# MattPlumlee/outerbase

Hardware: AMD Instinct MI355X
Metric: fit+predict points/sec, d=20 n=1e+06 p=4096 (higher is better)
Workload: dtype f64; 1 GPU; BASELINE.json configs[2]: d=20 n=1000000 (1000000 rows on each of 1 GPU(s)) p=4096, mat25, 40 knots/dim, fit (Gram+Cholesky) + predict on n fresh rows; backend=newton, rows_total=1000000, rows_per_gpu=1000000, d=20, p=4096, terms_nnz=12177, basis_columns=101, parallelism=one rank: nothing to exchange (y standardised first, one B^T y pass)

## Files before the change

outerbase_amd/csrc/kernels_gram_panel.hip:

```cpp
#include <algorithm>
#include <map>
#include <mutex>
#include <tuple>

#include <memory>
#include "obhip_internal.h"
#include "device_common.h"

namespace obhip {

namespace {

constexpr int kGT = 128;
constexpr int kCR = 16;
constexpr int kTP = 2 * 128 + 16;
constexpr int kTB = 65;

template <int W2>
__global__ void __launch_bounds__(256)
k_materialize_rows(const double *__restrict__ bm, const double *__restrict__ scale,
                   const uint32_t *__restrict__ ucol, int Mu, uint64_t Mc,
                   const uint32_t *__restrict__ colsw, int W2rt, uint64_t p_pad,
                   double *__restrict__ out) {
  extern __shared__ double lds[];
  double *tb = lds + (size_t)Mu * kTileRows;
  const int lane = threadIdx.x & 63;
  const int wave = __builtin_amdgcn_readfirstlane(threadIdx.x >> 6);
  const uint64_t tile = blockIdx.x;
  stage_tile<false, false>(lds, bm + tile * Mc * kTileRows, ucol, Mu, threadIdx.x, 256);
  __syncthreads();
  const double s = scale[tile * kTileRows + lane];
  double *mytb = tb + wave * 32 * kTB;
  const int ngroups = (int)(p_pad / 64);
  for (int g = wave; g < ngroups; g += 4) {
    const int k0 = g * 64;
    uint32_t cw[W2 > 0 ? W2 : 1];
    if constexpr (W2 > 0) load_cw(cw, colsw, k0 + lane);
#pragma unroll
    for (int h = 0; h < 2; ++h) {
#pragma unroll
      for (int t = 0; t < 32; ++t) {
        double v;
        if constexpr (W2 > 0)
          v = term_prod_rl<W2>(lds, cw, h * 32 + t, lane, s);
        else
          v = term_prod_mem(lds, colsw + (size_t)(k0 + h * 32 + t) * W2rt, W2rt, lane, s);
        mytb[t * kTB + lane] = v;
      }
      asm volatile("s_waitcnt lgkmcnt(0)" ::: "memory");
      double *dst = out + (tile * kTileRows + (lane >> 5)) * p_pad + k0 + h * 32 + (lane & 31);
      const double *src = mytb + (lane & 31) * kTB + (lane >> 5);
#pragma unroll 8
      for (int i = 0; i < 32; ++i) dst[(size_t)(2 * i) * p_pad] = src[2 * i];
      asm volatile("s_waitcnt lgkmcnt(0)" ::: "memory");
    }
  }
}

__device__ __forceinline__ void lds_dma_1k(const char *gbase , uint32_t voff,
                                           uint32_t lds_addr ) {
#pragma clang diagnostic push
#pragma clang diagnostic ignored "-Winline-asm"
  asm volatile("s_mov_b32 m0, %2\n\ts_nop 0\n\tglobal_load_lds_dwordx4 %0, %1"
               :: "v"(voff), "s"(gbase), "s"(lds_addr) : "memory", "m0");
#pragma clang diagnostic pop
}

template <int OFF>
__device__ __forceinline__ double lds_rd(uint32_t addr) {
  double v;
  asm volatile("ds_read_b64 %0, %1 offset:%2" : "=v"(v) : "v"(addr), "n"(OFF));
  return v;
}

__device__ __forceinline__ void lds_wait12(double (&a)[4], double (&b)[4][4]) {
  asm volatile("s_waitcnt lgkmcnt(8)"
               : "+v"(a[0]), "+v"(a[1]), "+v"(a[2]), "+v"(a[3]), "+v"(b[0][0]), "+v"(b[0][1]),
                 "+v"(b[0][2]), "+v"(b[0][3]), "+v"(b[1][0]), "+v"(b[1][1]), "+v"(b[1][2]),
                 "+v"(b[1][3]));
}
template <int KEEP>
__device__ __forceinline__ void lds_wait8(double (&b)[4][4]) {
  asm volatile("s_waitcnt lgkmcnt(%8)"
               : "+v"(b[2][0]), "+v"(b[2][1]), "+v"(b[2][2]), "+v"(b[2][3]), "+v"(b[3][0]),
                 "+v"(b[3][1]), "+v"(b[3][2]), "+v"(b[3][3])
               : "n"(KEEP));
}
template <int OFF>
__device__ __forceinline__ void lds_rd_h0(uint32_t aaddr, const uint32_t (&baddr)[4],
                                          double (&a)[4], double (&b)[4][4]) {
  a[0] = lds_rd<OFF>(aaddr);
  a[1] = lds_rd<OFF + 128>(aaddr);
  a[2] = lds_rd<OFF + 256>(aaddr);
  a[3] = lds_rd<OFF + 384>(aaddr);
#pragma unroll
  for (int r = 0; r < 4; ++r) {
    b[0][r] = lds_rd<OFF>(baddr[r]);
    b[1][r] = lds_rd<OFF + 128>(baddr[r]);
  }
}
template <int OFF>
__device__ __forceinline__ void lds_rd_h1(const uint32_t (&baddr)[4], double (&b)[4][4]) {
#pragma unroll
  for (int r = 0; r < 4; ++r) {
    b[2][r] = lds_rd<OFF + 256>(baddr[r]);
    b[3][r] = lds_rd<OFF + 384>(baddr[r]);
  }
}

constexpr int kAtbGram = 0, kAtbNorm = 1, kAtbStore = 2;
__host__ __device__ inline uint64_t atb_task(uint64_t I, uint64_t J, uint64_t y, uint64_t type = 0) {
  return I | (J << 24) | (y << 48) | (type << 62);
}
constexpr uint64_t kAtbNoTask = ~0ull;
__device__ __forceinline__ uint32_t atb_wave_code(uint32_t type, int wave) {
  constexpr uint32_t W = 0x80u;
  const uint32_t t0 = (W | 0x08u) | (W | 0x2cu) << 8 | (W | 0x19u) << 16 | (W | 0x3du) << 24;
  const uint32_t t1 = 0x00u | 0x24u << 8 | 0x35u << 16 | 0x4au << 24;
  const uint32_t t2 = 0x24u | 0x35u << 8 | 0x4au << 16 | 0x6eu << 24;
  const uint32_t t3 = 0x35u | 0x4au << 8 | 0x6eu << 16 | 0x7fu << 24;
  const uint32_t tab = type == 0 ? t0 : (type == 1 ? t1 : (type == 2 ? t2 : t3));
  return (tab >> (8 * wave)) & 0xffu;
}

template <int MODE, bool DBG>
__global__ void __launch_bounds__(256, 2)
k_atb_dma2(const double *__restrict__ A, uint64_t ldA, const double *__restrict__ Bm, uint64_t ldB,
           int nb, int npairs, uint64_t ntiles, uint64_t split_base ,
           int tri ,
           const uint64_t *__restrict__ tasks, double *__restrict__ part, uint64_t ldo,
           unsigned long long *dbgout) {
  extern __shared__ double T[];
  constexpr int tszb = kCR * kTP * 8;
  unsigned long long st0 = 0, sr0 = 0;
  if constexpr (DBG) {
    st0 = __builtin_amdgcn_s_memtime();
    sr0 = __builtin_amdgcn_s_memrealtime();
  }
  const int tid = threadIdx.x;
  const int lane = tid & 63;
  const int wave = __builtin_amdgcn_readfirstlane(tid >> 6);

  const uint64_t task = tasks[blockIdx.x];
  if (task == kAtbNoTask) return;
  const int I = (int)(task & 0xffffff), J = (int)((task >> 24) & 0xffffff), ysplit = (int)((task >> 48) & 0x3fff);
  const uint32_t wcode = atb_wave_code(MODE == kAtbGram ? (uint32_t)(task >> 62) : 0u, wave);

  uint64_t t0, t1;
  if constexpr (MODE == kAtbGram) {
    const uint64_t y = (uint64_t)ysplit, rem = (uint64_t)tri;
    t0 = y * split_base + min(y, rem);
    t1 = t0 + split_base + (y < rem ? 1 : 0);
  } else {
    t0 = 0;
    t1 = tri ? min(ntiles, (uint64_t)(J + 1) * (kGT / kTileRows)) : ntiles;
  }
  const int nchunks = (int)(t1 > t0 ? (t1 - t0) * (kTileRows / kCR) : 0);

  const uint32_t ldsT = (uint32_t)(uintptr_t)(__attribute__((address_space(3))) double *)T;
  const uint32_t lds0 = ldsT + wave * kTP * 8;
  const uint32_t voff = lane * 16;
  const char *gA = (const char *)(A + (t0 * kTileRows + wave) * ldA + (uint64_t)I * kGT);
  const char *gB = (const char *)(Bm + (t0 * kTileRows + wave) * ldB + (uint64_t)J * kGT);
  const uint64_t pitch4 = 4 * ldA * sizeof(double), pitch16 = 4 * pitch4;
  const uint64_t pitch4b = MODE == kAtbGram ? pitch4 : 4 * ldB * sizeof(double), pitch16b = 4 * pitch4b;
  const int rot = nchunks > 0 ? ((I + J) & 7) % nchunks : 0;
  auto issue = [&](int ch, int buf) {
    const uint32_t l = lds0 + buf * tszb;
    int cr = ch + rot;
    cr = cr >= nchunks ? cr - nchunks : cr;
    const char *a = gA + (uint64_t)cr * pitch16, *b = gB + (uint64_t)cr * pitch16b;
#pragma unroll
    for (int q = 0; q < 4; ++q) {
      lds_dma_1k(a + q * pitch4, voff, l + q * 4 * kTP * 8);
      lds_dma_1k(b + q * pitch4b, voff, l + q * 4 * kTP * 8 + kGT * 8);
    }
  };

  const int wm = (int)((wcode >> 4) & 1), wn = (int)((wcode >> 5) & 1);
  const int acol = (int)(wcode & 3) * 64, bcol = (int)((wcode >> 2) & 3) * 64;
  const int mk = lane >> 4, mblk = (lane >> 2) & 3, me = lane & 3;
  double acc[4][4][4];
#pragma unroll
  for (int i = 0; i < 4; ++i)
#pragma unroll
    for (int j = 0; j < 4; ++j)
#pragma unroll
      for (int r = 0; r < 4; ++r) acc[i][j][r] = 0.0;
  const uint32_t aaddr = ldsT + (mk * kTP + acol + mblk * 4 + me) * 8;
  uint32_t baddr[4];
#pragma unroll
  for (int r = 0; r < 4; ++r)
    baddr[r] = ldsT + (mk * kTP + bcol + ((mblk + r) & 3) * 4 + me) * 8;
  auto mfma_half = [&](const double (&a)[4], const double (&b)[4][4], int j0) {
#pragma unroll
    for (int i = 0; i < 4; ++i)
#pragma unroll
      for (int j = j0; j < j0 + 2; ++j)
#pragma unroll
        for (int r = 0; r < 4; ++r)
          acc[i][j][r] = __builtin_amdgcn_mfma_f64_4x4x4f64(a[i], b[j][r], acc[i][j][r], 0, 0, 0);
  };

  if (nchunks > 0) issue(0, 0);
  asm volatile("s_waitcnt vmcnt(0)" ::: "memory");
  __builtin_amdgcn_s_barrier();
  unsigned long long sr1 = 0, sr2 = 0;
  if constexpr (DBG) sr1 = __builtin_amdgcn_s_memrealtime();
  double a0[4], b0[4][4], a1[4], b1[4][4];
  constexpr int stp = 4 * kTP * 8;

#define OB_STEP(cur_a, cur_b, nxt_a, nxt_b, NEXT_OFF, HAS_NEXT)                              \
  lds_wait12(cur_a, cur_b);                                                               \
  if (HAS_NEXT) lds_rd_h0<NEXT_OFF>(aaddr, baddr, nxt_a, nxt_b);                             \
  mfma_half(cur_a, cur_b, 0);                                                                \
  lds_wait8<(HAS_NEXT) ? 12 : 0>(cur_b);                                                     \
  if (HAS_NEXT) lds_rd_h1<NEXT_OFF>(baddr, nxt_b);                                           \
  mfma_half(cur_a, cur_b, 2);

#define OB_CHUNK_BODY2(BUF)                                                                  \
  {                                                                                          \
    constexpr int ob = (BUF) * tszb;                                                         \
    if (c + 1 < nchunks) issue(c + 1, (BUF) ^ 1);                \
    lds_rd_h0<ob>(aaddr, baddr, a0, b0);                                                     \
    lds_rd_h1<ob>(baddr, b0);                                                                \
    OB_STEP(a0, b0, a1, b1, ob + stp, true)                                                  \
    OB_STEP(a1, b1, a0, b0, ob + 2 * stp, true)                                              \
    OB_STEP(a0, b0, a1, b1, ob + 3 * stp, true)                                              \
    OB_STEP(a1, b1, a0, b0, 0, false)                                                        \
    asm volatile("s_waitcnt vmcnt(0)" ::: "memory");     \
    __builtin_amdgcn_s_barrier();                                                            \
    ++c;                                                                                     \
  }

  for (int c = 0; c < nchunks;) {
    OB_CHUNK_BODY2(0)
    if (c >= nchunks) break;
    OB_CHUNK_BODY2(1)
  }
#undef OB_CHUNK_BODY2
#undef OB_STEP
  if constexpr (DBG) sr2 = __builtin_amdgcn_s_memrealtime();

  if constexpr (MODE == kAtbGram) {
    const int sel = (int)(wcode >> 6);
    const int oi = sel == 1 ? J : I, oj = sel == 0 ? I : J;
    const int slot = oi * nb - oi * (oi - 1) / 2 + (oj - oi);
    double *out = part + ((uint64_t)ysplit * npairs + slot) * (kGT * kGT);
#pragma unroll
    for (int i = 0; i < 4; ++i)
#pragma unroll
      for (int j = 0; j < 4; ++j)
#pragma unroll
        for (int r = 0; r < 4; ++r) {
          const int row = wm * 64 + i * 16 + mblk * 4 + mk;
          const int col = wn * 64 + j * 16 + ((mblk + r) & 3) * 4 + me;
          out[row * kGT + col] = acc[i][j][r];
        }
  } else if constexpr (MODE == kAtbStore) {
    double *out = part + ((uint64_t)I * kGT) * ldo + (uint64_t)J * kGT;
#pragma unroll
    for (int i = 0; i < 4; ++i)
#pragma unroll
      for (int j = 0; j < 4; ++j)
#pragma unroll
        for (int r = 0; r < 4; ++r) {
          const int row = wm * 64 + i * 16 + mblk * 4 + mk;
          const int col = wn * 64 + j * 16 + ((mblk + r) & 3) * 4 + me;
          out[(uint64_t)row * ldo + col] = acc[i][j][r];
        }
  } else {
    double *red = T;
#pragma unroll
    for (int i = 0; i < 4; ++i) {
      double s = 0.0;
#pragma unroll
      for (int j = 0; j < 4; ++j)
#pragma unroll
        for (int r = 0; r < 4; ++r) s = fma(acc[i][j][r], acc[i][j][r], s);
      s += __shfl_xor(s, 1, 64);
      s += __shfl_xor(s, 2, 64);
      if (me == 0) red[wn * kGT + wm * 64 + i * 16 + mblk * 4 + mk] = s;
    }
    __syncthreads();
    if (tid < kGT) part[(uint64_t)J * ldo + (uint64_t)I * kGT + tid] = red[tid] + red[kGT + tid];
  }
  if constexpr (DBG) {
    const unsigned which = blockIdx.x == 7 ? 1u : blockIdx.x == gridDim.x / 2 + 7 ? 0u
                           : blockIdx.x + 512 - 7 == gridDim.x - (gridDim.x % 512 ? gridDim.x % 512 : 0) ? 2u : 3u;
    if (dbgout && which < 3 && tid == 0) {
      dbgout[3 * which] = __builtin_amdgcn_s_memtime() - st0;
      dbgout[3 * which + 1] = __builtin_amdgcn_s_memrealtime() - sr0;
      dbgout[3 * which + 2] = nchunks;
    }
    const bool mid0 = blockIdx.x == gridDim.x / 2 + 7, mid1 = blockIdx.x == gridDim.x / 2 + 7 + 512;
    if (dbgout && (mid0 || mid1) && tid == 0) {
      asm volatile("s_waitcnt vmcnt(0)" ::: "memory");
      unsigned long long *o = dbgout + 9 + (mid1 ? 4 : 0);
      o[0] = sr0;
      o[1] = sr1;
      o[2] = sr2;
      o[3] = __builtin_amdgcn_s_memrealtime();
    }
  }
}

constexpr int kXcd = 8, kSq = 8;
struct GramUnit {
  int bi, bj, y, size;
};
void gram_units(int nb, int nsplit, bool diag4, std::vector<GramUnit> &units) {
  const int nsq = (nb + kSq - 1) / kSq;
  for (int y = 0; y < nsplit; ++y)
    for (int bi = 0; bi < nsq; ++bi)
      for (int bj = bi; bj < nsq; ++bj) {
        int size = 0;
        for (int i = bi * kSq; i < std::min(nb, (bi + 1) * kSq); ++i)
          for (int j = std::max(i, bj * kSq); j < std::min(nb, (bj + 1) * kSq); ++j)
            if (!(i == j && diag4 && i / 4 * 4 + 3 < nb && i % 4 == 3)) ++size;
        if (size) units.push_back({bi, bj, y, size});
      }
}
uint64_t gram_xcd_blocks(int nb, int nsplit, bool diag4, bool continuous) {
  std::vector<GramUnit> units;
  gram_units(nb, 1, diag4, units);
  uint64_t per_split = 0;
  for (const GramUnit &u : units) per_split += (uint64_t)u.size;
  if (continuous) return (per_split * (uint64_t)nsplit + kXcd - 1) / kXcd;
  std::vector<int> sizes;
  for (int y = 0; y < nsplit; ++y)
    for (const GramUnit &u : units) sizes.push_back(u.size);
  std::stable_sort(sizes.begin(), sizes.end(), [](int a, int b) { return a > b; });
  uint64_t load[kXcd] = {0};
  for (int s : sizes) {
    int k = 0;
    for (int q = 1; q < kXcd; ++q)
      if (load[q] < load[k]) k = q;
    load[k] += (uint64_t)s;
  }
  return *std::max_element(load, load + kXcd);
}
void build_task_order(int nb, int nsplit, bool diag4, bool continuous, std::vector<uint64_t> &tab) {
  typedef GramUnit Unit;
  std::vector<Unit> units;
  gram_units(nb, nsplit, diag4, units);
  if (!continuous)
    std::stable_sort(units.begin(), units.end(), [](const Unit &a, const Unit &b) { return a.size > b.size; });
  uint64_t total = 0;
  for (const Unit &u : units) total += (uint64_t)u.size;
  const uint64_t run = (total + kXcd - 1) / kXcd;
  uint64_t dealt = 0;
  std::vector<std::vector<uint64_t>> seq(kXcd);
  for (const Unit &u : units) {
    int k = 0;
    for (int q = 1; q < kXcd; ++q)
      if (seq[q].size() < seq[k].size()) k = q;
    if (continuous) {
      for (int i = u.bi * kSq; i < std::min(nb, (u.bi + 1) * kSq); ++i)
        for (int j = std::max(i, u.bj * kSq); j < std::min(nb, (u.bj + 1) * kSq); ++j) {
          if (i == j && diag4) {
            const int g0 = i / 4 * 4;
            if (g0 + 3 < nb) {
              if (i - g0 < 3) seq[(dealt++) / run].push_back(atb_task(i, i + 1, u.y, 1 + (i - g0)));
              continue;
            }
          }
          seq[(dealt++) / run].push_back(atb_task(i, j, u.y));
        }
      continue;
    }
    for (int i = u.bi * kSq; i < std::min(nb, (u.bi + 1) * kSq); ++i)
      for (int j = std::max(i, u.bj * kSq); j < std::min(nb, (u.bj + 1) * kSq); ++j) {
        if (i == j && diag4) {
          const int g0 = i / 4 * 4;
          if (g0 + 3 < nb) {
            if (i - g0 < 3) seq[k].push_back(atb_task(i, i + 1, u.y, 1 + (i - g0)));
            continue;
          }
        }
        seq[k].push_back(atb_task(i, j, u.y));
      }
  }
  size_t len = 0;
  for (auto &q : seq) len = std::max(len, q.size());
  tab.assign(len * kXcd, kAtbNoTask);
  for (int k = 0; k < kXcd; ++k)
    for (size_t m = 0; m < seq[k].size(); ++m) tab[m * kXcd + k] = seq[k][m];
}

template <int W2>
int run_materialize(const obhip_basis &b, obhip_terms &t, double *d_B) {
  const size_t lds = (t.Mu * kTileRows + 4 * 32 * kTB) * sizeof(double);
  OB_TRY(ensure_dyn_lds((const void *)k_materialize_rows<W2>, lds));
  hipLaunchKernelGGL(k_materialize_rows<W2>, dim3((unsigned)(b.n_pad / kTileRows)), dim3(256), lds,
                     cur_stream(), b.bm.p, b.scale.p, t.ucol.p, (int)t.Mu, b.md.Mc,
                     (const uint32_t *)t.cols.p, (int)(t.W / 2), t.p_pad, d_B);
  OB_HIP(hipGetLastError());
  return 0;
}

}

bool gram_panel_supports(const obhip_basis &b, const obhip_terms &t) {
  const size_t need = (size_t)b.n_pad * t.p_pad * sizeof(double);
  if (b.bmat.n * sizeof(double) >= need) return true;
  if (getenv("OBHIP_GRAM_CHUNK_ROWS")) return false;
  size_t free_b = 0, total_b = 0;
  if (hipMemGetInfo(&free_b, &total_b) != hipSuccess) return false;
  return need <= free_b / 2;
}

namespace {

struct RowView {
  obhip_basis v;
  RowView(const obhip_basis &b, uint64_t tile0, uint64_t ntiles) {
    v.model = b.model;
    v.d = b.d;
    v.device = b.device;
    v.md.Mc = b.md.Mc;
    v.n_pad = ntiles * kTileRows;
    const uint64_t r0 = tile0 * kTileRows;
    v.n = r0 >= b.n ? 0 : std::min<uint64_t>(v.n_pad, b.n - r0);
    v.bm.p = b.bm.p + tile0 * b.md.Mc * kTileRows;
    v.scale.p = b.scale.p + r0;
  }
  ~RowView() {
    v.bm.p = nullptr;
    v.scale.p = nullptr;
  }
};

int materialize_any(const obhip_basis &b, obhip_terms &t, double *d_B, GramFuse *fuse = nullptr) {
  if (t.Mu > 280 || getenv("OBHIP_FORCE_GENERIC")) return launch_materialize_generic(b, t, d_B);
  static const bool lane_row = getenv("OBHIP_MATERIALIZE_LANE_ROW") != nullptr;
  if (!lane_row && materialize_tl_supports(t)) {
    const bool f = fuse && fuse->y && fuse->g && !fuse->done;
    OB_TRY(launch_materialize_tl(b, t, d_B, f ? fuse->y : nullptr, f ? fuse->g : nullptr));
    if (f) fuse->done = true;
    return 0;
  }
  switch (t.W / 2) {
    case 1: return run_materialize<1>(b, t, d_B);
    case 2: return run_materialize<2>(b, t, d_B);
    case 3: return run_materialize<3>(b, t, d_B);
    case 4: return run_materialize<4>(b, t, d_B);
    default: return run_materialize<0>(b, t, d_B);
  }
}

int gram_of_staged(obhip_basis &b, const double *d_B, uint64_t ntiles, obhip_terms &t,
                   const GramSink &sink, bool accumulate, bool last) {
  const bool dbg = getenv("OBHIP_GRAM_DBG") && atoi(getenv("OBHIP_GRAM_DBG")) != 0;
  const int nb = (int)((t.p + kGT - 1) / kGT);
  const int npairs = nb * (nb + 1) / 2;
  const int ncu = device_cus(b.device);
  const bool diag4 = !(getenv("OBHIP_GRAM_DIAG4") && atoi(getenv("OBHIP_GRAM_DIAG4")) == 0);
  const uint64_t bps = (uint64_t)npairs - (diag4 ? (uint64_t)(nb / 4) : 0);
  const uint64_t slots = 2 * (uint64_t)ncu;
  uint64_t nsplit = 1;
  const uint64_t max_split = std::max<uint64_t>(
      1, std::min<uint64_t>({64, ntiles / 8, (4ull << 30) / ((uint64_t)npairs * kGT * kGT * 8)}));
  double bestc = 1e300;
  bool continuous = false;
  const uint64_t xslots = slots / kXcd;
  static std::mutex split_mu;
  static std::map<std::tuple<int, uint64_t, uint64_t, uint64_t, bool>, std::pair<uint64_t, bool>> split_cache;
  const auto split_key = std::make_tuple(nb, ntiles, max_split, slots, diag4);
  bool cached = false;
  {
    std::lock_guard<std::mutex> lk(split_mu);
    auto it = split_cache.find(split_key);
    if (it != split_cache.end()) {
      nsplit = it->second.first;
      continuous = it->second.second;
      cached = true;
    }
  }
  for (uint64_t ns = 1; !cached && ns <= max_split; ++ns) {
    const uint64_t blocks = ns * bps;
    for (int mode = 0; mode < 2; ++mode) {
      const uint64_t per = gram_xcd_blocks(nb, (int)ns, diag4, mode == 1);
      const uint64_t full = per / xslots, tail = per % xslots;
      const double rounds = (double)full + (tail == 0 ? 0.0 : (2 * tail <= xslots ? 0.6 : 1.0));
      double cost = rounds * ((double)ntiles / (double)ns + 1.0) + 0.0022 * (double)blocks;
      if (mode == 1) cost *= 1.03;
      if (cost < bestc - 1e-9) {
        bestc = cost;
        nsplit = ns;
        continuous = mode == 1;
      }
    }
  }
  if (!cached) {
    std::lock_guard<std::mutex> lk(split_mu);
    split_cache[split_key] = std::make_pair(nsplit, continuous);
  }
  if (const char *e = getenv("OBHIP_GRAM_NSPLIT")) nsplit = std::max<uint64_t>(1, std::min<uint64_t>(max_split, atoi(e)));
  if (const char *e = getenv("OBHIP_GRAM_CONTINUOUS")) continuous = atoi(e) != 0;
  double *part = nullptr;
  OB_TRY(b.workspace((size_t)nsplit * npairs * kGT * kGT * sizeof(double) + 256, (void **)&part));
  unsigned long long *dbgout =
      dbg ? (unsigned long long *)(part + (size_t)nsplit * npairs * kGT * kGT) : nullptr;
  if (b.gram_pairs_nb != nb || b.gram_pairs_ns != (int)nsplit || b.gram_pairs_diag4 != diag4 ||
      b.gram_pairs_cont != continuous) {
    std::vector<uint64_t> tab;
    build_task_order(nb, (int)nsplit, diag4, continuous, tab);
    b.gram_pairs_diag4 = diag4;
    b.gram_pairs_cont = continuous;
    OB_TRY(b.gram_pairs.upload(tab.data(), tab.size()));
    b.gram_pairs_nb = nb;
    b.gram_pairs_ns = (int)nsplit;
  }
  const unsigned nblocks = (unsigned)b.gram_pairs.n;
  const size_t lds = (size_t)2 * kCR * kTP * sizeof(double);
  {
    ProfScope ps("gram");
    if (dbg) {
      OB_TRY(ensure_dyn_lds((const void *)k_atb_dma2<kAtbGram, true>, lds));
      hipLaunchKernelGGL((k_atb_dma2<kAtbGram, true>), dim3(nblocks), dim3(256), lds, cur_stream(), d_B,
                         t.p_pad, d_B, t.p_pad, nb, npairs, ntiles, ntiles / nsplit, (int)(ntiles % nsplit), b.gram_pairs.p, part,
                         (uint64_t)0, dbgout);
    } else {
      OB_TRY(ensure_dyn_lds((const void *)k_atb_dma2<kAtbGram, false>, lds));
      hipLaunchKernelGGL((k_atb_dma2<kAtbGram, false>), dim3(nblocks), dim3(256), lds, cur_stream(),
                         d_B, t.p_pad, d_B, t.p_pad, nb, npairs, ntiles, ntiles / nsplit, (int)(ntiles % nsplit), b.gram_pairs.p, part,
                         (uint64_t)0, nullptr);
    }
    OB_HIP(hipGetLastError());
  }
  if (dbgout) {
    unsigned long long h[17];
    OB_HIP(hipMemcpy(h, dbgout, sizeof(h), hipMemcpyDeviceToHost));
    fprintf(stderr, "[gram dbg] middle-round block: first chunk %.2f us, loop %.2f us, stores %.2f us; the block one round "
                    "on starts %.2f us after this one ended (its first chunk %.2f us)\n",
            0.01 * (double)(h[10] - h[9]), 0.01 * (double)(h[11] - h[10]), 0.01 * (double)(h[12] - h[11]),
            0.01 * (double)((long long)h[13] - (long long)h[12]), 0.01 * (double)(h[14] - h[13]));
    fprintf(stderr, "[gram dbg] clock of a block of the first / middle / last round: %.0f / %.0f / %.0f MHz\n",
            h[4] ? 100.0 * h[3] / h[4] : 0.0, h[1] ? 100.0 * h[0] / h[1] : 0.0, h[7] ? 100.0 * h[6] / h[7] : 0.0);
    fprintf(stderr,
            "[gram dbg] one block: %llu shader-clock ticks in %llu x 10 ns -> %.0f MHz, %.0f ticks "
            "per 16-row chunk (8192 = matrix pipe saturated by two blocks)\n",
            h[0], h[1], h[1] ? 100.0 * h[0] / h[1] : 0.0, h[2] ? (double)h[0] / h[2] : 0.0);
  }
  return launch_gram_reduce(part, npairs, (int)nsplit, nb, (int)t.p, sink, accumulate, last);
}

}

int launch_materialize_rows(const obhip_basis &b, obhip_terms &t, double *d_B, GramFuse *fuse) {
  OB_TRY(t.prepare(b.md.cap, b.md.dims_h));
  ProfScope ps("materialize_B");
  return materialize_any(b, t, d_B, fuse);
}

int ensure_bmat(obhip_basis &b, obhip_terms &t, GramFuse *fuse) {
  if (b.bmat_terms == t.uid && t.uid != 0) return 0;
  OB_TRY(t.prepare(b.md.cap, b.md.dims_h));
  if (!gram_panel_supports(b, t))
    return fail(OBHIP_ERR_INVALID, "not enough free HBM for the n x p design matrix");
  const size_t need = (size_t)b.n_pad * t.p_pad;
  if (b.bmat.n < need) OB_TRY(b.bmat.alloc(need));
  b.bmat_terms = 0;
  OB_TRY(launch_materialize_rows(b, t, b.bmat.p, fuse));
  b.bmat_terms = t.uid;
  return 0;
}

int launch_gram_panel(const obhip_basis &bc, obhip_terms &t, const GramSink &sink, GramFuse *fuse) {
  obhip_basis &b = const_cast<obhip_basis &>(bc);
  const uint64_t ntiles = b.n_pad / kTileRows;
  if (gram_panel_supports(b, t)) {
    OB_TRY(ensure_bmat(b, t, fuse));
    return gram_of_staged(b, b.bmat.p, ntiles, t, sink, false, true);
  }
  size_t free_b = 0, total_b = 0;
  OB_HIP(hipMemGetInfo(&free_b, &total_b));
  const size_t row_bytes = (size_t)t.p_pad * kTileRows * sizeof(double);
  uint64_t ctiles = std::min<size_t>(free_b / 4, (size_t)16 << 30) / row_bytes;
  if (const char *e = getenv("OBHIP_GRAM_CHUNK_ROWS")) ctiles = (uint64_t)atoll(e) / kTileRows;
  ctiles = std::max<uint64_t>(ctiles, 1);
  ctiles = std::min(ctiles, ntiles);
  if ((size_t)ctiles * row_bytes > free_b)
    return fail(OBHIP_ERR_HIP, "not enough free HBM for even one row chunk of the design matrix");
  b.bmat_terms = 0;
  if (b.bmat.n < (size_t)ctiles * kTileRows * t.p_pad) OB_TRY(b.bmat.alloc((size_t)ctiles * kTileRows * t.p_pad));
  static const bool overlap = getenv("OBHIP_GRAM_OVERLAP") && atoi(getenv("OBHIP_GRAM_OVERLAP")) != 0;
  if (overlap && ctiles < ntiles) {
    DevBuf<double> second;
    OB_TRY(second.alloc((size_t)ctiles * kTileRows * t.p_pad));
    hipStream_t mainst = cur_stream(), side = nullptr;
    OB_HIP(hipStreamCreateWithFlags(&side, hipStreamNonBlocking));
    hipEvent_t ev0, evM[2], evG[2];
    OB_HIP(hipEventCreateWithFlags(&ev0, hipEventDisableTiming));
    for (int i = 0; i < 2; ++i) {
      OB_HIP(hipEventCreateWithFlags(&evM[i], hipEventDisableTiming));
      OB_HIP(hipEventCreateWithFlags(&evG[i], hipEventDisableTiming));
    }
    OB_HIP(hipEventRecord(ev0, mainst));
    OB_HIP(hipStreamWaitEvent(side, ev0, 0));
    int rc = 0;
    uint64_t c = 0;
    for (uint64_t t0 = 0; t0 < ntiles && rc == 0; t0 += ctiles, ++c) {
      const uint64_t nt = std::min(ctiles, ntiles - t0);
      const int buf = (int)(c & 1);
      double *Bp = buf ? second.p : b.bmat.p;
      RowView view(b, t0, nt);
      if (c >= 2) (void)hipStreamWaitEvent(side, evG[buf], 0);
      set_cur_stream(side);
      {
        ProfScope ps("materialize_B");
        rc = materialize_any(view.v, t, Bp);
      }
      (void)hipEventRecord(evM[buf], side);
      set_cur_stream(mainst);
      if (rc) break;
      (void)hipStreamWaitEvent(mainst, evM[buf], 0);
      rc = gram_of_staged(b, Bp, nt, t, sink, t0 != 0, t0 + nt >= ntiles);
      (void)hipEventRecord(evG[buf], mainst);
    }
    (void)hipStreamSynchronize(side);
    (void)hipStreamSynchronize(mainst);
    (void)hipEventDestroy(ev0);
    for (int i = 0; i < 2; ++i) {
      (void)hipEventDestroy(evM[i]);
      (void)hipEventDestroy(evG[i]);
    }
    (void)hipStreamDestroy(side);
    return rc;
  }
  for (uint64_t t0 = 0; t0 < ntiles; t0 += ctiles) {
    const uint64_t nt = std::min(ctiles, ntiles - t0);
    RowView view(b, t0, nt);
    {
      ProfScope ps("materialize_B");
      OB_TRY(materialize_any(view.v, t, b.bmat.p));
    }
    OB_TRY(gram_of_staged(b, b.bmat.p, nt, t, sink, t0 != 0, t0 + nt >= ntiles));
  }
  return 0;
}

int launch_atb(int mode, const double *A, uint64_t ldA, uint64_t M, const double *Bm, uint64_t ldB,
               uint64_t N, uint64_t K, bool tri, double *out, uint64_t ldo) {
  if (M % kGT || N % kGT || K % kTileRows)
    return fail(OBHIP_ERR_INVALID, "launch_atb: sizes must be padded to the tile");
  const uint64_t mt = M / kGT, nt = N / kGT;
  if (mt >= (1ull << 24) || nt >= (1ull << 24)) return fail(OBHIP_ERR_INVALID, "launch_atb: too many tiles");
  constexpr size_t kAtbCache = 8;
  using Tab = std::shared_ptr<DevBuf<uint64_t>>;
  static std::mutex mu;
  static std::map<std::tuple<int, uint64_t, uint64_t>, Tab> cache;
  static std::vector<std::tuple<int, uint64_t, uint64_t>> lru;
  int dev = 0;
  (void)hipGetDevice(&dev);
  Tab dtabp, victim;
  int victim_dev = dev;
  {
    std::lock_guard<std::mutex> lk(mu);
    const auto key = std::make_tuple(dev, mt, nt);
    lru.erase(std::remove(lru.begin(), lru.end(), key), lru.end());
    lru.push_back(key);
    if (lru.size() > kAtbCache) {
      auto it = cache.find(lru.front());
      if (it != cache.end()) {
        victim = std::move(it->second);
        victim_dev = std::get<0>(lru.front());
        cache.erase(it);
      }
      lru.erase(lru.begin());
    }
    Tab &slot = cache[key];
    if (!slot) {
      std::vector<std::vector<uint64_t>> seq(kXcd);
      for (uint64_t bj = 0; bj * kSq < nt; ++bj)
        for (uint64_t bi = 0; bi * kSq < mt; ++bi) {
          int k = 0;
          for (int q = 1; q < kXcd; ++q)
            if (seq[q].size() < seq[k].size()) k = q;
          for (uint64_t i = bi * kSq; i < std::min(mt, (bi + 1) * kSq); ++i)
            for (uint64_t j = bj * kSq; j < std::min(nt, (bj + 1) * kSq); ++j) seq[k].push_back(atb_task(i, j, 0));
        }
      size_t len = 0;
      for (auto &q : seq) len = std::max(len, q.size());
      std::vector<uint64_t> tab(len * kXcd, kAtbNoTask);
      for (int k = 0; k < kXcd; ++k)
        for (size_t m = 0; m < seq[k].size(); ++m) tab[m * kXcd + k] = seq[k][m];
      slot = std::make_shared<DevBuf<uint64_t>>();
      const int rc = slot->upload(tab.data(), tab.size());
      if (rc) {
        cache.erase(key);
        lru.pop_back();
        return rc;
      }
    }
    dtabp = slot;
  }
  if (victim) {
    if (victim_dev != dev) (void)hipSetDevice(victim_dev);
    (void)hipDeviceSynchronize();
    victim.reset();
    if (victim_dev != dev) (void)hipSetDevice(dev);
  }
  DevBuf<uint64_t> &dtab = *dtabp;
  const size_t ntasks = dtab.n;
  const size_t lds = (size_t)2 * kCR * kTP * sizeof(double);
  const uint64_t ktiles = K / kTileRows;
  if (mode == kAtbNorm) {
    OB_TRY(ensure_dyn_lds((const void *)k_atb_dma2<kAtbNorm, false>, lds));
    hipLaunchKernelGGL((k_atb_dma2<kAtbNorm, false>), dim3((unsigned)ntasks), dim3(256), lds,
                       cur_stream(), A, ldA, Bm, ldB, 0, 0, ktiles, ktiles, tri ? 1 : 0, dtab.p, out,
                       ldo, nullptr);
  } else if (mode == kAtbStore) {
    OB_TRY(ensure_dyn_lds((const void *)k_atb_dma2<kAtbStore, false>, lds));
    hipLaunchKernelGGL((k_atb_dma2<kAtbStore, false>), dim3((unsigned)ntasks), dim3(256), lds,
                       cur_stream(), A, ldA, Bm, ldB, 0, 0, ktiles, ktiles, tri ? 1 : 0, dtab.p, out,
                       ldo, nullptr);
  } else {
    return fail(OBHIP_ERR_INVALID, "launch_atb: unknown mode");
  }
  OB_HIP(hipGetLastError());
  return 0;
}

}
```

Baseline: 4.159 million points/s.

## Skip redundant lower-triangle MFMAs in packed diagonal Gram tiles

For Gram tasks that pack four diagonal tile pairs into one block, each wave now gets a role that computes only the upper-triangle MFMAs it owns, plus a few extra rows to rebalance work across waves. It mirrors the needed diagonal entries on store. The split-count cost model is also told how much work this saves. This cuts matrix-pipe work on diagonal blocks, at the price of a second specialised inner loop, more code and register pressure, and a complex ownership mapping guarded by compile-time coverage checks.

```diff
diff --git a/outerbase_amd/csrc/kernels_gram_panel.hip b/outerbase_amd/csrc/kernels_gram_panel.hip
--- a/outerbase_amd/csrc/kernels_gram_panel.hip
+++ b/outerbase_amd/csrc/kernels_gram_panel.hip
@@ -113,7 +113,7 @@
   return I | (J << 24) | (y << 48) | (type << 62);
 }
 constexpr uint64_t kAtbNoTask = ~0ull;
-__device__ __forceinline__ uint32_t atb_wave_code(uint32_t type, int wave) {
+__host__ __device__ constexpr uint32_t atb_wave_code(uint32_t type, int wave) {
   constexpr uint32_t W = 0x80u;
   const uint32_t t0 = (W | 0x08u) | (W | 0x2cu) << 8 | (W | 0x19u) << 16 | (W | 0x3du) << 24;
   const uint32_t t1 = 0x00u | 0x24u << 8 | 0x35u << 16 | 0x4au << 24;
@@ -123,12 +123,179 @@
   return (tab >> (8 * wave)) & 0xffu;
 }
 
+constexpr int kTriMain = 0, kTriD2 = 1, kTriD4 = 2, kTriO10 = 3, kTriO12 = 4;
+constexpr int kTriLen13 = 44, kTriLen2 = 52;
+__host__ __device__ constexpr bool tri_is_d(int kind) { return kind == kTriD2 || kind == kTriD4; }
+__host__ __device__ constexpr bool tri_d_own(int i, int j, int r) { return i < j || (i == j && r < 3); }
+__host__ __device__ constexpr int tri_extra_rows(int kind) { return kind == kTriD2 ? 2 : (kind == kTriD4 ? 4 : 0); }
+__host__ __device__ constexpr bool tri_o_keeps(int kind, int i, int j) {
+  return j >= 2 || (j == 1 && (kind == kTriO12 || i >= 2));
+}
+__host__ __device__ constexpr uint32_t tri_role_byte(int kind, int src = 0, int i0 = 0, int j = 0) {
+  return (uint32_t)kind | (uint32_t)src << 3 | (uint32_t)(i0 >> 1) << 4 | (uint32_t)j << 5;
+}
+__host__ __device__ constexpr uint32_t tri_role(uint32_t type, int wave) {
+  const uint32_t t1 = tri_role_byte(kTriD2, 0, 0, 0) | tri_role_byte(kTriO10) << 8 |
+                      tri_role_byte(kTriD2, 0, 2, 0) << 16 | tri_role_byte(kTriD2, 0, 0, 1) << 24;
+  const uint32_t t2 = tri_role_byte(kTriO12) | tri_role_byte(kTriD4, 0, 0, 0) << 8 |
+                      tri_role_byte(kTriD4, 1, 0, 0) << 16 | tri_role_byte(kTriO12) << 24;
+  const uint32_t t3 = tri_role_byte(kTriD2, 1, 0, 0) | tri_role_byte(kTriD2, 1, 2, 0) << 8 |
+                      tri_role_byte(kTriO10) << 16 | tri_role_byte(kTriD2, 1, 0, 1) << 24;
+  const uint32_t tab = type == 0 ? 0u : (type == 1 ? t1 : (type == 2 ? t2 : t3));
+  return (tab >> (8 * wave)) & 0xffu;
+}
+__host__ __device__ constexpr int tri_role_mfmas(int kind) {
+  int n = 0;
+  for (int i = 0; i < 4; ++i)
+    for (int j = 0; j < 4; ++j)
+      for (int r = 0; r < 4; ++r) n += tri_is_d(kind) ? (tri_d_own(i, j, r) ? 1 : 0) : (tri_o_keeps(kind, i, j) ? 1 : 0);
+  return n + 4 * tri_extra_rows(kind);
+}
+static_assert(tri_role_mfmas(kTriD2) == kTriLen13 && tri_role_mfmas(kTriO10) == 40, "types 1, 3: 44 44 44 40");
+static_assert(tri_role_mfmas(kTriD4) == kTriLen2 && tri_role_mfmas(kTriO12) == 48, "type 2: 48 52 52 48");
+__host__ __device__ constexpr bool tri_cover_ok(uint32_t type, int want_mfmas) {
+  int cnt[2][32][32] = {}, want[2][32][32] = {};
+  int mfmas = 0;
+  for (int w = 0; w < 4; ++w) {
+    const uint32_t code = atb_wave_code(type, w), role = tri_role(type, w);
+    const int sel = (int)(code >> 6), wm = (int)((code >> 4) & 1), wn = (int)((code >> 5) & 1);
+    const int kind = (int)(role & 7);
+    if (sel > 1 || kind == kTriMain) return false;
+    if (tri_is_d(kind) != ((code & 3) == ((code >> 2) & 3))) return false;
+    mfmas += tri_role_mfmas(kind);
+    for (int br = 0; br < 16; ++br)
+      for (int bc = 0; bc < 16; ++bc)
+        if (wn * 16 + bc >= wm * 16 + br) ++want[sel][wm * 16 + br][wn * 16 + bc];
+    for (int i = 0; i < 4; ++i)
+      for (int j = 0; j < 4; ++j)
+        for (int r = 0; r < 4; ++r)
+          for (int blk = 0; blk < 4; ++blk) {
+            if (!(tri_is_d(kind) ? tri_d_own(i, j, r) : tri_o_keeps(kind, i, j))) continue;
+            const int gr = wm * 16 + i * 4 + blk, gc = wn * 16 + j * 4 + ((blk + r) & 3);
+            if (gc >= gr)
+              ++cnt[sel][gr][gc];
+            else if (i == j && r == 1 && blk == 3)
+              ++cnt[sel][gc][gr];
+          }
+    if (tri_is_d(kind)) {
+      const int src = (int)((role >> 3) & 1), i0 = (int)((role >> 4) & 1) * 2, ej = (int)((role >> 5) & 1);
+      for (int k = 0; k < tri_extra_rows(kind); ++k)
+        for (int r = 0; r < 4; ++r)
+          for (int blk = 0; blk < 4; ++blk) ++cnt[src][(i0 + k) * 4 + blk][16 + ej * 4 + ((blk + r) & 3)];
+    }
+  }
+  for (int s = 0; s < 2; ++s)
+    for (int a = 0; a < 32; ++a)
+      for (int b = 0; b < 32; ++b)
+        if (cnt[s][a][b] != want[s][a][b]) return false;
+  return mfmas == want_mfmas;
+}
+static_assert(tri_role(0, 0) == kTriMain && tri_role(0, 1) == kTriMain && tri_role(0, 2) == kTriMain &&
+                  tri_role(0, 3) == kTriMain,
+              "a whole tile pair (type 0) has no roles");
+static_assert(tri_cover_ok(1, 3 * 36 + 64) && tri_cover_ok(2, 2 * 36 + 2 * 64) && tri_cover_ok(3, 3 * 36 + 64),
+              "role tables of the packed diagonal blocks");
+
+struct TriOps {
+  double a[4], b[4][4], ea[4], eb[4];
+};
+template <int KIND>
+struct TriCut {
+  static constexpr bool D = tri_is_d(KIND);
+  static constexpr int nea = tri_extra_rows(KIND);
+  static constexpr int n0 = D ? 11 : 12, n1 = D ? 8 + nea : 4;
+  static_assert(n0 <= 15 && n1 <= 15, "lgkmcnt holds 4 bits");
+};
+template <int KIND, int OFF>
+__device__ __forceinline__ void tri_rd_h0(uint32_t aaddr, const uint32_t (&baddr)[4], TriOps &o) {
+  if constexpr (TriCut<KIND>::D) {
+#pragma unroll
+    for (int r = 0; r < 3; ++r) o.b[0][r] = lds_rd<OFF>(baddr[r]);
+#pragma unroll
+    for (int r = 0; r < 4; ++r) o.b[1][r] = lds_rd<OFF + 128>(baddr[r]);
+#pragma unroll
+    for (int r = 0; r < 4; ++r) o.b[2][r] = lds_rd<OFF + 256>(baddr[r]);
+  } else {
+    o.a[0] = lds_rd<OFF>(aaddr);
+    o.a[1] = lds_rd<OFF + 128>(aaddr);
+    o.a[2] = lds_rd<OFF + 256>(aaddr);
+    o.a[3] = lds_rd<OFF + 384>(aaddr);
+#pragma unroll
+    for (int r = 0; r < 4; ++r) o.b[1][r] = lds_rd<OFF + 128>(baddr[r]);
+#pragma unroll
+    for (int r = 0; r < 4; ++r) o.b[2][r] = lds_rd<OFF + 256>(baddr[r]);
+  }
+}
+template <int KIND, int OFF>
+__device__ __forceinline__ void tri_rd_h1(const uint32_t (&baddr)[4], uint32_t eaaddr,
+                                          const uint32_t (&ebaddr)[4], TriOps &o) {
+#pragma unroll
+  for (int r = 0; r < 4; ++r) o.b[3][r] = lds_rd<OFF + 384>(baddr[r]);
+  if constexpr (TriCut<KIND>::D) {
+    o.ea[0] = lds_rd<OFF>(eaaddr);
+    o.ea[1] = lds_rd<OFF + 128>(eaaddr);
+    if constexpr (TriCut<KIND>::nea == 4) {
+      o.ea[2] = lds_rd<OFF + 256>(eaaddr);
+      o.ea[3] = lds_rd<OFF + 384>(eaaddr);
+    }
+#pragma unroll
+    for (int r = 0; r < 4; ++r) o.eb[r] = lds_rd<OFF>(ebaddr[r]);
+  }
+}
+__device__ __forceinline__ void tri_tie(double &x) { asm volatile("" : "+v"(x)); }
+template <int KIND, int HALF, int KEEP>
+__device__ __forceinline__ void tri_wait(TriOps &o) {
+  asm volatile("s_waitcnt lgkmcnt(%0)" ::"n"(KEEP));
+  constexpr bool D = TriCut<KIND>::D;
+  if constexpr (HALF == 0) {
+    if constexpr (!D) {
+#pragma unroll
+      for (int i = 0; i < 4; ++i) tri_tie(o.a[i]);
+    }
+#pragma unroll
+    for (int j = D ? 0 : 1; j < 3; ++j)
+#pragma unroll
+      for (int r = 0; r < 4; ++r)
+        if (!(D && j == 0 && r == 3)) tri_tie(o.b[j][r]);
+  } else {
+#pragma unroll
+    for (int r = 0; r < 4; ++r) tri_tie(o.b[3][r]);
+    if constexpr (D) {
+#pragma unroll
+      for (int k = 0; k < TriCut<KIND>::nea; ++k) tri_tie(o.ea[k]);
+#pragma unroll
+      for (int r = 0; r < 4; ++r) tri_tie(o.eb[r]);
+    }
+  }
+}
+template <int KIND, int HALF>
+__device__ __forceinline__ void tri_mfma(const TriOps &o, double (&acc)[4][4][4], double (&xacc)[4][4]) {
+  constexpr bool D = TriCut<KIND>::D;
+#pragma unroll
+  for (int j = HALF == 0 ? 0 : 3; j < (HALF == 0 ? 3 : 4); ++j)
+#pragma unroll
+    for (int i = 0; i < 4; ++i)
+#pragma unroll
+      for (int r = 0; r < 4; ++r) {
+        if (D ? tri_d_own(i, j, r) : tri_o_keeps(KIND, i, j))
+          acc[i][j][r] = __builtin_amdgcn_mfma_f64_4x4x4f64(D ? o.b[i][0] : o.a[i], o.b[j][r], acc[i][j][r], 0, 0, 0);
+      }
+  if constexpr (D && HALF == 1) {
+#pragma unroll
+    for (int k = 0; k < TriCut<KIND>::nea; ++k)
+#pragma unroll
+      for (int r = 0; r < 4; ++r)
+        xacc[k][r] = __builtin_amdgcn_mfma_f64_4x4x4f64(o.ea[k], o.eb[r], xacc[k][r], 0, 0, 0);
+  }
+}
+
 template <int MODE, bool DBG>
 __global__ void __launch_bounds__(256, 2)
 k_atb_dma2(const double *__restrict__ A, uint64_t ldA, const double *__restrict__ Bm, uint64_t ldB,
            int nb, int npairs, uint64_t ntiles, uint64_t split_base ,
            int tri ,
            const uint64_t *__restrict__ tasks, double *__restrict__ part, uint64_t ldo,
+           int diagtri ,
            unsigned long long *dbgout) {
   extern __shared__ double T[];
   constexpr int tszb = kCR * kTP * 8;
@@ -145,6 +312,7 @@
   if (task == kAtbNoTask) return;
   const int I = (int)(task & 0xffffff), J = (int)((task >> 24) & 0xffffff), ysplit = (int)((task >> 48) & 0x3fff);
   const uint32_t wcode = atb_wave_code(MODE == kAtbGram ? (uint32_t)(task >> 62) : 0u, wave);
+  const uint32_t role = MODE == kAtbGram && diagtri ? tri_role((uint32_t)(task >> 62), wave) : 0u;
 
   uint64_t t0, t1;
   if constexpr (MODE == kAtbGram) {
@@ -210,6 +378,95 @@
   double a0[4], b0[4][4], a1[4], b1[4][4];
   constexpr int stp = 4 * kTP * 8;
 
+  bool tri_done = false;
+  if constexpr (MODE == kAtbGram) {
+    auto tri_run = [&](auto kind_c) {
+      constexpr int KIND = decltype(kind_c)::value;
+      constexpr bool D = TriCut<KIND>::D;
+      constexpr int nea = TriCut<KIND>::nea, n0 = TriCut<KIND>::n0, n1 = TriCut<KIND>::n1;
+      const int src = (int)((role >> 3) & 1), ei0 = (int)((role >> 4) & 1) * 2, ej = (int)((role >> 5) & 1);
+      const uint32_t eaaddr = ldsT + (mk * kTP + src * kGT + ei0 * 16 + mblk * 4 + me) * 8;
+      uint32_t ebaddr[4];
+#pragma unroll
+      for (int r = 0; r < 4; ++r)
+        ebaddr[r] = ldsT + (mk * kTP + src * kGT + 64 + ej * 16 + ((mblk + r) & 3) * 4 + me) * 8;
+      double tacc[4][4][4], xacc[4][4];
+#pragma unroll
+      for (int i = 0; i < 4; ++i)
+#pragma unroll
+        for (int j = 0; j < 4; ++j) {
+          xacc[i][j] = 0.0;
+#pragma unroll
+          for (int r = 0; r < 4; ++r) tacc[i][j][r] = 0.0;
+        }
+      TriOps o0, o1;
+#define OB_TRI_STEP(cur, nxt, NEXT_OFF, HAS_NEXT)                                            \
+  tri_wait<KIND, 0, n1>(cur);                                                                \
+  if (HAS_NEXT) tri_rd_h0<KIND, NEXT_OFF>(aaddr, baddr, nxt);                                \
+  tri_mfma<KIND, 0>(cur, tacc, xacc);                                                        \
+  tri_wait<KIND, 1, (HAS_NEXT) ? n0 : 0>(cur);                                               \
+  if (HAS_NEXT) tri_rd_h1<KIND, NEXT_OFF>(baddr, eaaddr, ebaddr, nxt);                       \
+  tri_mfma<KIND, 1>(cur, tacc, xacc);
+#define OB_TRI_CHUNK(BUF)                                                                    \
+  {                                                                                          \
+    constexpr int ob = (BUF) * tszb;                                                         \
+    if (c + 1 < nchunks) issue(c + 1, (BUF) ^ 1);                                            \
+    tri_rd_h0<KIND, ob>(aaddr, baddr, o0);                                                   \
+    tri_rd_h1<KIND, ob>(baddr, eaaddr, ebaddr, o0);                                          \
+    OB_TRI_STEP(o0, o1, ob + stp, true)                                                      \
+    OB_TRI_STEP(o1, o0, ob + 2 * stp, true)                                                  \
+    OB_TRI_STEP(o0, o1, ob + 3 * stp, true)                                                  \
+    OB_TRI_STEP(o1, o0, 0, false)                                                            \
+    asm volatile("s_waitcnt vmcnt(0)" ::: "memory");                                         \
+    __builtin_amdgcn_s_barrier();                                                            \
+    ++c;                                                                                     \
+  }
+      for (int c = 0; c < nchunks;) {
+        OB_TRI_CHUNK(0)
+        if (c >= nchunks) break;
+        OB_TRI_CHUNK(1)
+      }
+#undef OB_TRI_CHUNK
+#undef OB_TRI_STEP
+      const int sel = (int)(wcode >> 6);
+      const int ot = sel == 1 ? J : I;
+      double *out = part + ((uint64_t)ysplit * npairs + (ot * nb - ot * (ot - 1) / 2)) * (kGT * kGT);
+#pragma unroll
+      for (int i = 0; i < 4; ++i)
+#pragma unroll
+        for (int j = 0; j < 4; ++j)
+#pragma unroll
+          for (int r = 0; r < 4; ++r) {
+            if (!(D ? tri_d_own(i, j, r) : tri_o_keeps(KIND, i, j))) continue;
+            const int row = wm * 64 + i * 16 + mblk * 4 + mk;
+            const int col = wn * 64 + j * 16 + ((mblk + r) & 3) * 4 + me;
+            out[row * kGT + col] = tacc[i][j][r];
+            if (D && i == j && r == 1 && mblk == 3) out[col * kGT + row] = tacc[i][j][r];
+          }
+      if constexpr (D) {
+        const int xt = src ? J : I;
+        double *xout = part + ((uint64_t)ysplit * npairs + (xt * nb - xt * (xt - 1) / 2)) * (kGT * kGT);
+#pragma unroll
+        for (int k = 0; k < nea; ++k)
+#pragma unroll
+          for (int r = 0; r < 4; ++r) {
+            const int row = (ei0 + k) * 16 + mblk * 4 + mk;
+            const int col = 64 + ej * 16 + ((mblk + r) & 3) * 4 + me;
+            xout[row * kGT + col] = xacc[k][r];
+          }
+      }
+    };
+    if (role != 0) {
+      switch (role & 7) {
+        case kTriD2: tri_run(std::integral_constant<int, kTriD2>()); break;
+        case kTriD4: tri_run(std::integral_constant<int, kTriD4>()); break;
+        case kTriO10: tri_run(std::integral_constant<int, kTriO10>()); break;
+        default: tri_run(std::integral_constant<int, kTriO12>()); break;
+      }
+      tri_done = true;
+    }
+  }
+
 #define OB_STEP(cur_a, cur_b, nxt_a, nxt_b, NEXT_OFF, HAS_NEXT)                              \
   lds_wait12(cur_a, cur_b);                                                               \
   if (HAS_NEXT) lds_rd_h0<NEXT_OFF>(aaddr, baddr, nxt_a, nxt_b);                             \
@@ -233,11 +490,12 @@
     ++c;                                                                                     \
   }
 
-  for (int c = 0; c < nchunks;) {
-    OB_CHUNK_BODY2(0)
-    if (c >= nchunks) break;
-    OB_CHUNK_BODY2(1)
-  }
+  if (!tri_done)
+    for (int c = 0; c < nchunks;) {
+      OB_CHUNK_BODY2(0)
+      if (c >= nchunks) break;
+      OB_CHUNK_BODY2(1)
+    }
 #undef OB_CHUNK_BODY2
 #undef OB_STEP
   if constexpr (DBG) sr2 = __builtin_amdgcn_s_memrealtime();
@@ -247,16 +505,18 @@
     const int oi = sel == 1 ? J : I, oj = sel == 0 ? I : J;
     const int slot = oi * nb - oi * (oi - 1) / 2 + (oj - oi);
     double *out = part + ((uint64_t)ysplit * npairs + slot) * (kGT * kGT);
-#pragma unroll
-    for (int i = 0; i < 4; ++i)
-#pragma unroll
-      for (int j = 0; j < 4; ++j)
-#pragma unroll
-        for (int r = 0; r < 4; ++r) {
-          const int row = wm * 64 + i * 16 + mblk * 4 + mk;
-          const int col = wn * 64 + j * 16 + ((mblk + r) & 3) * 4 + me;
-          out[row * kGT + col] = acc[i][j][r];
-        }
+    if (!tri_done) {
+#pragma unroll
+      for (int i = 0; i < 4; ++i)
+#pragma unroll
+        for (int j = 0; j < 4; ++j)
+#pragma unroll
+          for (int r = 0; r < 4; ++r) {
+            const int row = wm * 64 + i * 16 + mblk * 4 + mk;
+            const int col = wn * 64 + j * 16 + ((mblk + r) & 3) * 4 + me;
+            out[row * kGT + col] = acc[i][j][r];
+          }
+    }
   } else if constexpr (MODE == kAtbStore) {
     double *out = part + ((uint64_t)I * kGT) * ldo + (uint64_t)J * kGT;
 #pragma unroll
@@ -308,42 +568,57 @@
 constexpr int kXcd = 8, kSq = 8;
 struct GramUnit {
   int bi, bj, y, size;
+  int work;
 };
-void gram_units(int nb, int nsplit, bool diag4, std::vector<GramUnit> &units) {
+void gram_units(int nb, int nsplit, bool diag4, bool diagtri, std::vector<GramUnit> &units) {
   const int nsq = (nb + kSq - 1) / kSq;
   for (int y = 0; y < nsplit; ++y)
     for (int bi = 0; bi < nsq; ++bi)
       for (int bj = bi; bj < nsq; ++bj) {
-        int size = 0;
+        int size = 0, work = 0;
         for (int i = bi * kSq; i < std::min(nb, (bi + 1) * kSq); ++i)
-          for (int j = std::max(i, bj * kSq); j < std::min(nb, (bj + 1) * kSq); ++j)
-            if (!(i == j && diag4 && i / 4 * 4 + 3 < nb && i % 4 == 3)) ++size;
-        if (size) units.push_back({bi, bj, y, size});
+          for (int j = std::max(i, bj * kSq); j < std::min(nb, (bj + 1) * kSq); ++j) {
+            const bool packed = i == j && diag4 && i / 4 * 4 + 3 < nb;
+            if (packed && i % 4 == 3) continue;
+            ++size;
+            work += packed && diagtri ? (i % 4 == 1 ? kTriLen2 : kTriLen13) : 64;
+          }
+        if (size) units.push_back({bi, bj, y, size, work});
       }
 }
-uint64_t gram_xcd_blocks(int nb, int nsplit, bool diag4, bool continuous) {
+uint64_t gram_xcd_blocks(int nb, int nsplit, bool diag4, bool diagtri, bool continuous, double *saved) {
   std::vector<GramUnit> units;
-  gram_units(nb, 1, diag4, units);
-  uint64_t per_split = 0;
-  for (const GramUnit &u : units) per_split += (uint64_t)u.size;
-  if (continuous) return (per_split * (uint64_t)nsplit + kXcd - 1) / kXcd;
-  std::vector<int> sizes;
+  gram_units(nb, 1, diag4, diagtri, units);
+  uint64_t per_split = 0, work_split = 0;
+  for (const GramUnit &u : units) {
+    per_split += (uint64_t)u.size;
+    work_split += (uint64_t)u.work;
+  }
+  if (continuous) {
+    *saved = (double)(per_split * 64 - work_split) * (double)nsplit / (64.0 * kXcd);
+    return (per_split * (uint64_t)nsplit + kXcd - 1) / kXcd;
+  }
+  std::vector<std::pair<int, int>> sizes;
   for (int y = 0; y < nsplit; ++y)
-    for (const GramUnit &u : units) sizes.push_back(u.size);
-  std::stable_sort(sizes.begin(), sizes.end(), [](int a, int b) { return a > b; });
-  uint64_t load[kXcd] = {0};
-  for (int s : sizes) {
+    for (const GramUnit &u : units) sizes.push_back(std::make_pair(u.size, u.work));
+  std::stable_sort(sizes.begin(), sizes.end(),
+                   [](const std::pair<int, int> &a, const std::pair<int, int> &b) { return a.first > b.first; });
+  uint64_t load[kXcd] = {0}, work[kXcd] = {0};
+  for (const auto &s : sizes) {
     int k = 0;
     for (int q = 1; q < kXcd; ++q)
       if (load[q] < load[k]) k = q;
-    load[k] += (uint64_t)s;
-  }
-  return *std::max_element(load, load + kXcd);
+    load[k] += (uint64_t)s.first;
+    work[k] += (uint64_t)s.second;
+  }
+  const int k = (int)(std::max_element(load, load + kXcd) - load);
+  *saved = (double)(load[k] * 64 - work[k]) / 64.0;
+  return load[k];
 }
 void build_task_order(int nb, int nsplit, bool diag4, bool continuous, std::vector<uint64_t> &tab) {
   typedef GramUnit Unit;
   std::vector<Unit> units;
-  gram_units(nb, nsplit, diag4, units);
+  gram_units(nb, nsplit, diag4, false, units);
   if (!continuous)
     std::stable_sort(units.begin(), units.end(), [](const Unit &a, const Unit &b) { return a.size > b.size; });
   uint64_t total = 0;
@@ -456,6 +731,7 @@
   const int npairs = nb * (nb + 1) / 2;
   const int ncu = device_cus(b.device);
   const bool diag4 = !(getenv("OBHIP_GRAM_DIAG4") && atoi(getenv("OBHIP_GRAM_DIAG4")) == 0);
+  const bool diagtri = diag4 && !(getenv("OBHIP_GRAM_DIAGTRI") && atoi(getenv("OBHIP_GRAM_DIAGTRI")) == 0);
   const uint64_t bps = (uint64_t)npairs - (diag4 ? (uint64_t)(nb / 4) : 0);
   const uint64_t slots = 2 * (uint64_t)ncu;
   uint64_t nsplit = 1;
@@ -465,8 +741,8 @@
   bool continuous = false;
   const uint64_t xslots = slots / kXcd;
   static std::mutex split_mu;
-  static std::map<std::tuple<int, uint64_t, uint64_t, uint64_t, bool>, std::pair<uint64_t, bool>> split_cache;
-  const auto split_key = std::make_tuple(nb, ntiles, max_split, slots, diag4);
+  static std::map<std::tuple<int, uint64_t, uint64_t, uint64_t, bool, bool>, std::pair<uint64_t, bool>> split_cache;
+  const auto split_key = std::make_tuple(nb, ntiles, max_split, slots, diag4, diagtri);
   bool cached = false;
   {
     std::lock_guard<std::mutex> lk(split_mu);
@@ -480,9 +756,10 @@
   for (uint64_t ns = 1; !cached && ns <= max_split; ++ns) {
     const uint64_t blocks = ns * bps;
     for (int mode = 0; mode < 2; ++mode) {
-      const uint64_t per = gram_xcd_blocks(nb, (int)ns, diag4, mode == 1);
+      double saved = 0.0;
+      const uint64_t per = gram_xcd_blocks(nb, (int)ns, diag4, diagtri, mode == 1, &saved);
       const uint64_t full = per / xslots, tail = per % xslots;
-      const double rounds = (double)full + (tail == 0 ? 0.0 : (2 * tail <= xslots ? 0.6 : 1.0));
+      const double rounds = (double)full + (tail == 0 ? 0.0 : (2 * tail <= xslots ? 0.6 : 1.0)) - saved / (double)xslots;
       double cost = rounds * ((double)ntiles / (double)ns + 1.0) + 0.0022 * (double)blocks;
       if (mode == 1) cost *= 1.03;
       if (cost < bestc - 1e-9) {
@@ -520,12 +797,12 @@
       OB_TRY(ensure_dyn_lds((const void *)k_atb_dma2<kAtbGram, true>, lds));
       hipLaunchKernelGGL((k_atb_dma2<kAtbGram, true>), dim3(nblocks), dim3(256), lds, cur_stream(), d_B,
                          t.p_pad, d_B, t.p_pad, nb, npairs, ntiles, ntiles / nsplit, (int)(ntiles % nsplit), b.gram_pairs.p, part,
-                         (uint64_t)0, dbgout);
+                         (uint64_t)0, diagtri ? 1 : 0, dbgout);
     } else {
       OB_TRY(ensure_dyn_lds((const void *)k_atb_dma2<kAtbGram, false>, lds));
       hipLaunchKernelGGL((k_atb_dma2<kAtbGram, false>), dim3(nblocks), dim3(256), lds, cur_stream(),
                          d_B, t.p_pad, d_B, t.p_pad, nb, npairs, ntiles, ntiles / nsplit, (int)(ntiles % nsplit), b.gram_pairs.p, part,
-                         (uint64_t)0, nullptr);
+                         (uint64_t)0, diagtri ? 1 : 0, nullptr);
     }
     OB_HIP(hipGetLastError());
   }
@@ -710,12 +987,12 @@
     OB_TRY(ensure_dyn_lds((const void *)k_atb_dma2<kAtbNorm, false>, lds));
     hipLaunchKernelGGL((k_atb_dma2<kAtbNorm, false>), dim3((unsigned)ntasks), dim3(256), lds,
                        cur_stream(), A, ldA, Bm, ldB, 0, 0, ktiles, ktiles, tri ? 1 : 0, dtab.p, out,
-                       ldo, nullptr);
+                       ldo, 0, nullptr);
   } else if (mode == kAtbStore) {
     OB_TRY(ensure_dyn_lds((const void *)k_atb_dma2<kAtbStore, false>, lds));
     hipLaunchKernelGGL((k_atb_dma2<kAtbStore, false>), dim3((unsigned)ntasks), dim3(256), lds,
                        cur_stream(), A, ldA, Bm, ldB, 0, 0, ktiles, ktiles, tri ? 1 : 0, dtab.p, out,
-                       ldo, nullptr);
+                       ldo, 0, nullptr);
   } else {
     return fail(OBHIP_ERR_INVALID, "launch_atb: unknown mode");
   }
```

Measured after the change: 4.008 million points/s. -3.6%, worse.
